# XiandaGuo/OpenStereo

Measured on NVIDIA H100. Metric: stereo_pairs_per_sec_gwcnet_256x512_d192, higher is better.
Workload: dtype f32

## Files before the change

### include/openstereo_b200.h

```cpp
#ifndef OPENSTEREO_B200_H_
#define OPENSTEREO_B200_H_

#include <stddef.h>
#include <stdint.h>

#ifdef __cplusplus
extern "C" {
#endif

#define OSB_OK 0
#define OSB_EINVAL 1
#define OSB_ECUDA 2
#define OSB_EUNSUPPORTED 3

#define OSB_ACT_NONE 0
#define OSB_ACT_RELU 1
#define OSB_ACT_LEAKY 2
#define OSB_ACT_RELU6 3

typedef void* osb_stream_t;

int osb_abi_version(void);
const char* osb_last_error(void);
uint64_t osb_launch_count(void);
// ... 39 lines not shown

int osb_deconv3d_bn_act_fwd(const float* x, const float* w_packed, const float* scale,
                            const float* shift, const float* residual, float* y, int B, int Cin,
                            int Cout, int D, int H, int W, int kernel, int act, osb_stream_t stream);

int osb_conv3d_1x1_bn_act_fwd(const float* x0, const float* x1, int Cin0, const float* w_packed,
                              const float* scale, const float* shift, const float* residual,
                              const float* gate, float* y, int B, int Cin, int Cout, int D, int H,
                              int W, int act, int sigmoid_out, osb_stream_t stream);


int osb_conv3d_tc_supported(int Cin, int Cout, int W, int stride);
#define OSB_TC_MIN_WIDTH 24
int osb_tc_general_width(int W);
int osb_conv3d_tc_kc(int Cin, int Cout, int W, int stride);
int osb_conv3d_k3_tc_fwd(const float* x_ndhwc, const void* w_split, const float* scale, const float* shift,
                         const float* residual, float* y, int B, int Cin, int Cout, int D, int H, int W, int act,
                         int out_ndhwc, int res_ndhwc, osb_stream_t stream);
int osb_conv3d_k3_tc_gate_fwd(const float* x_ndhwc, const void* w_split, const float* scale, const float* shift,
                              const float* residual, const float* gate_nhwc, float* y, int B, int Cin, int Cout, int D, int H, int W,
                              int act, osb_stream_t stream);
int osb_conv3d_k3_tc_ncdhw_fwd(const float* x_ncdhw, const void* w_split, const float* scale, const float* shift,
                               const float* residual, float* y, int B, int Cin, int Cout, int D, int H, int W, int act,
                               int out_ndhwc, int res_ndhwc, osb_stream_t stream);
int osb_conv3d_s2_tc_supported(int Cin, int Cout, int D, int H, int W);
int osb_conv3d_k3_s2_tc_fwd(const float* x_ndhwc, const void* w_split, const float* scale, const float* shift,
                            const float* residual, float* y, int B, int Cin, int Cout, int D, int H, int W, int act,
                            int out_ndhwc, int res_ndhwc, osb_stream_t stream);
int osb_deconv3d_tc_supported(int Cin, int Cout, int W);
int osb_deconv3d_k3_tc_fwd(const float* x_ndhwc, const void* w_split, const float* scale, const float* shift,
                           const float* residual, float* y, int B, int Cin, int Cout, int D, int H, int W, int act,
                           int out_ndhwc, int res_ndhwc, osb_stream_t stream);
int osb_deconv3d_k4_tc_supported(int Cin, int Cout, int W);
int osb_deconv3d_k4_tc_fwd(const float* x_ndhwc, const void* w_split, const float* scale, const float* shift,
                           const float* residual, float* y, int B, int Cin, int Cout, int cout_real, int D, int H, int W, int act,
                           int out_ndhwc, int res_ndhwc, osb_stream_t stream);
int osb_conv3d_k3_tc_cs_fwd(const float* x_ndhwc, const void* w_split, const float* scale, const float* shift, const float* residual,
                            const float* gate_nhwc, float* y, int B, int Cin, int Cout, int D, int H, int W, int act, int ystride,
                            osb_stream_t stream);
int osb_conv3d_k3_s2_tc_cs_fwd(const float* x_ndhwc, const void* w_split, const float* scale, const float* shift, float* y, int B,
                               int Cin, int Cout, int D, int H, int W, int act, int ystride, osb_stream_t stream);
int osb_deconv3d_k4_tc_cs_fwd(const float* x_ndhwc, const void* w_split, const float* scale, const float* shift, float* y, int B,
                              int Cin, int Cout, int D, int H, int W, int act, int ystride, osb_stream_t stream);
int osb_conv1x1_ndhwc_cat_fwd(const float* x0, const float* x1, int C0, int C1, const float* w_packed, const float* scale,
                              const float* shift, float* y, long long voxels, int Cout, int act, osb_stream_t stream);
int osb_conv1x1_ndhwc_fwd(const float* x, const float* w_packed, const float* scale, const float* shift, float* y,
                          long long voxels, int Cin, int Cout, int act, osb_stream_t stream);
int osb_conv3d_k3_c1_ndhwc_fwd(const float* x_ndhwc, const float* w_taps, const float* scale, const float* shift, float* y, int B,
                               int Cin, int D, int H, int W, osb_stream_t stream);
int osb_conv2d_tc_kc(int Cin, int Cout, int W, int dilation);
int osb_conv2d_k3_tc_fwd(const float* x_nhwc, const void* w_split, const float* scale, const float* shift, const float* residual,
                         float* y, int B, int Cin, int Cout, int H, int W, int dilation, int act, int out_nhwc, int res_nhwc,
                         osb_stream_t stream);
int osb_gwc_volume_sum_fwd(const float* ref, const float* tgt, float* out, int B, int C, int H, int W, int D, int G,
                           osb_stream_t stream);
int osb_group_l2_normalize_fwd(const float* x, float* y, int B, int C, int H, int W, int G, float eps, osb_stream_t stream);
int osb_sub_volume_fwd(const float* left, const float* right, float* out, int B, int C, int H, int W, int D, osb_stream_t stream);
int osb_regression_values_fwd(const float* prob, const float* values, float* out, int B, int D, int H, int W, osb_stream_t stream);

int osb_warped_concat_volume_fwd(const float* x, const float* y, const float* disp, float* out, int B, int C, int D, int H, int W,
                                 int mask_left, osb_stream_t stream);
int osb_warped_gwc_concat_volume_fwd(const float* xg, const float* yg, const float* xc, const float* yc, const float* disp,
                                     float* out, int B, int Cg, int G, int Cc, int D, int H, int W, osb_stream_t stream);

int osb_coex_regression_fwd(const float* cost, const float* spx, float* out, int B, int D, int h, int w, int top_k, int spx_is_logits,
                            osb_stream_t stream);
int osb_nearest_resize3d_fwd(const float* x, float* y, int N, int Di, int Hi, int Wi, int Do, int Ho, int Wo, osb_stream_t stream);

int osb_mbv2_block3d_fwd(const float* x, const float* w_exp, const float* scale1, const float* shift1, const float* w_dw,
                         const float* scale2, const float* shift2, const float* w_proj, const float* scale3, const float* shift3,
                         const float* residual, float* y, int B, int Cin, int Chid, int Cout, int D, int H, int W, int stride,
                         int in_layout, int out_layout, osb_stream_t stream);

int osb_gwc_volume_bwd(const float* grad_vol, const float* ref, const float* tgt, float* grad_ref, float* grad_tgt, int B, int C,
                       int H, int W, int D, int G, int reduce_sum, osb_stream_t stream);
int osb_concat_volume_bwd(const float* grad_vol, float* grad_ref, float* grad_tgt, int B, int C, int H, int W, int D, int mask_left,
                          osb_stream_t stream);
int osb_softargmin_bwd(const float* cost, const float* grad_out, float* grad_cost, int B, int D, int H, int W, float alpha,
                       float start, float step, int normalize, osb_stream_t stream);

int osb_dwconv2d_fwd(const float* x, const float* w, const float* scale, const float* shift, const float* residual, float* y, int B,
                     int C, int H, int W, int KH, int KW, int stride, int act, osb_stream_t stream);
int osb_deconv2d_k3s2_fwd(const float* x, const float* w_packed, const float* scale, const float* shift, const float* residual,
                          float* y, int B, int Cin, int Cout, int H, int W, int act, osb_stream_t stream);

int osb_avgpool_pairs_fwd(const float* x, float* y, long long outer, int n, long long inner, osb_stream_t stream);
int osb_geo_lookup_fwd(const float* geo0, const float* geo1, const float* geo2, const float* geo3, const float* corr0,
                       const float* corr1, const float* corr2, const float* corr3, const float* disp, const float* coords,
                       float* out, int B, int C, int D, int H, int W, int W2, int num_levels, int radius, osb_stream_t stream);
int osb_context_upsample_fwd(const float* disp_low, const float* up_weights, float* out, int B, int h, int w, int scale,
                             osb_stream_t stream);
int osb_ncdhw_to_ndhwc(const float* x, float* y, int B, int C, int D, int H, int W, osb_stream_t stream);
int osb_ncdhw_to_ndhwc_pad(const float* x, float* y, int B, int C, int Cpad, int D, int H, int W, osb_stream_t stream);
int osb_feature_att_gate_fwd(const float* feat_nchw, const float* w1_packed, const float* scale1, const float* shift1,
                             const float* w2_packed, const float* scale2, const float* shift2, float* gate_nhwc, int B,
                             int Cf, int Ch, int Cv, int Cpad, int HW, int act1, osb_stream_t stream);

#ifdef __cplusplus
}
#endif
#endif
```

### openstereo_b200/_lib.py

```python
import ctypes
import os

_PKG = os.path.dirname(os.path.abspath(__file__))
LIB_PATH = os.path.join(_PKG, "lib", "libopenstereo_b200.so")

_f32p = ctypes.c_void_p
_i = ctypes.c_int
_f = ctypes.c_float
_s = ctypes.c_void_p

SIGNATURES = {
    "osb_gwc_volume_fwd": [_f32p, _f32p, _f32p, _i, _i, _i, _i, _i, _i, _s],
    "osb_concat_volume_fwd": [_f32p, _f32p, _f32p, _i, _i, _i, _i, _i, _i, _s],
    "osb_gwc_concat_volume_fwd": [_f32p, _f32p, _f32p, _f32p, _f32p, _i, _i, _i, _i, _i, _i, _i, _s],
    "osb_corr_volume_fwd": [_f32p, _f32p, _f32p, _i, _i, _i, _i, _i, _s],
    "osb_softargmin_fwd": [_f32p, _f32p, _i, _i, _i, _i, _f, _f, _f, _i, _s],
    "osb_upsample_softargmin_fwd": [_f32p, _f32p, _i, _i, _i, _i, _i, _i, _i, _i, _s],
    "osb_epe_partial_fwd": [_f32p, _f32p, _f32p, _i, _i, _f, _s],
    "osb_conv3d_k3_bn_act_fwd": [_f32p] * 7 + [_i] * 8 + [_s],
    "osb_deconv3d_bn_act_fwd": [_f32p] * 6 + [_i] * 8 + [_s],
    "osb_conv3d_1x1_bn_act_fwd": [_f32p, _f32p, _i] + [_f32p] * 6 + [_i] * 8 + [_s],
    "osb_conv3d_tc_supported": [_i, _i, _i, _i],
    "osb_conv3d_tc_kc": [_i, _i, _i, _i],
    "osb_tc_general_width": [_i],
    "osb_conv3d_s2_tc_supported": [_i, _i, _i, _i, _i],
    "osb_deconv3d_tc_supported": [_i, _i, _i],
    "osb_deconv3d_k3_tc_fwd": [_f32p] * 6 + [_i] * 9 + [_s],
    "osb_conv3d_k3_s2_tc_fwd": [_f32p] * 6 + [_i] * 9 + [_s],
    "osb_conv3d_k3_tc_fwd": [_f32p] * 6 + [_i] * 9 + [_s],
    "osb_conv3d_k3_tc_ncdhw_fwd": [_f32p] * 6 + [_i] * 9 + [_s],
    "osb_conv3d_k3_tc_gate_fwd": [_f32p] * 7 + [_i] * 7 + [_s],
    "osb_deconv3d_k4_tc_supported": [_i, _i, _i],
    "osb_conv3d_k3_tc_cs_fwd": [_f32p] * 7 + [_i] * 8 + [_s],
    "osb_conv3d_k3_s2_tc_cs_fwd": [_f32p] * 5 + [_i] * 8 + [_s],
    "osb_deconv3d_k4_tc_cs_fwd": [_f32p] * 5 + [_i] * 8 + [_s],
    "osb_deconv3d_k4_tc_fwd": [_f32p] * 6 + [_i] * 10 + [_s],
    "osb_conv1x1_ndhwc_cat_fwd": [_f32p, _f32p, _i, _i, _f32p, _f32p, _f32p, _f32p, ctypes.c_longlong, _i, _i, _s],
    "osb_feature_att_gate_fwd": [_f32p] * 8 + [_i] * 7 + [_s],
    "osb_ncdhw_to_ndhwc_pad": [_f32p, _f32p, _i, _i, _i, _i, _i, _i, _s],
    "osb_conv1x1_ndhwc_fwd": [_f32p] * 5 + [ctypes.c_longlong, _i, _i, _i, _s],
    "osb_conv3d_k3_c1_ndhwc_fwd": [_f32p] * 5 + [_i] * 5 + [_s],
    "osb_avgpool_pairs_fwd": [_f32p, _f32p, ctypes.c_longlong, _i, ctypes.c_longlong, _s],
    "osb_geo_lookup_fwd": [_f32p] * 11 + [_i] * 8 + [_s],
    "osb_context_upsample_fwd": [_f32p] * 3 + [_i] * 4 + [_s],
    "osb_conv2d_tc_kc": [_i] * 4,
    "osb_conv2d_k3_tc_fwd": [_f32p] * 6 + [_i] * 9 + [_s],
    "osb_ncdhw_to_ndhwc": [_f32p, _f32p, _i, _i, _i, _i, _i, _s],
    "osb_gwc_volume_sum_fwd": [_f32p, _f32p, _f32p, _i, _i, _i, _i, _i, _i, _s],
    "osb_group_l2_normalize_fwd": [_f32p, _f32p, _i, _i, _i, _i, _i, _f, _s],
    "osb_sub_volume_fwd": [_f32p, _f32p, _f32p, _i, _i, _i, _i, _i, _s],
    "osb_regression_values_fwd": [_f32p, _f32p, _f32p, _i, _i, _i, _i, _s],
    "osb_gwc_volume_bwd": [_f32p] * 5 + [_i] * 7 + [_s],
    "osb_concat_volume_bwd": [_f32p] * 3 + [_i] * 6 + [_s],
    "osb_softargmin_bwd": [_f32p] * 3 + [_i] * 4 + [_f, _f, _f, _i, _s],
    "osb_dwconv2d_fwd": [_f32p] * 6 + [_i] * 8 + [_s],
    "osb_deconv2d_k3s2_fwd": [_f32p] * 6 + [_i] * 6 + [_s],
    "osb_upsample_softargmin_values_fwd": [_f32p] * 3 + [_i] * 8 + [_s],
    "osb_warped_concat_volume_fwd": [_f32p] * 4 + [_i] * 6 + [_s],
    "osb_warped_gwc_concat_volume_fwd": [_f32p] * 6 + [_i] * 7 + [_s],
    "osb_coex_regression_fwd": [_f32p] * 3 + [_i] * 6 + [_s],
    "osb_nearest_resize3d_fwd": [_f32p] * 2 + [_i] * 7 + [_s],
    "osb_mbv2_block3d_fwd": [_f32p] * 12 + [_i] * 10 + [_s],
}


class NativeLibraryError(RuntimeError):
    pass


def _load():
    if not os.path.exists(LIB_PATH):
        raise NativeLibraryError(
            "%s not found: build it with `python -m openstereo_b200.build` (there is no CPU/PyTorch fallback)"
            % LIB_PATH)
    lib = ctypes.CDLL(LIB_PATH)
    lib.osb_abi_version.restype = ctypes.c_int
    lib.osb_last_error.restype = ctypes.c_char_p
    lib.osb_launch_count.restype = ctypes.c_uint64
    lib.osb_tc_overflow_count.argtypes = [ctypes.c_void_p, ctypes.c_int, ctypes.POINTER(ctypes.c_uint)]
    lib.osb_tc_overflow_count.restype = ctypes.c_int
    lib.osb_tc_overflow_poll.argtypes = [ctypes.c_void_p, ctypes.c_void_p]
    lib.osb_tc_overflow_poll.restype = ctypes.c_int
    lib.osb_tc_overflow_flag.argtypes = []
    lib.osb_tc_overflow_flag.restype = ctypes.c_void_p
    lib.osb_set_rz_kappa.argtypes = [ctypes.c_float]
    lib.osb_set_rz_kappa.restype = ctypes.c_float
    lib.osb_set_persistent_grid_cap.argtypes = [ctypes.c_int]
    lib.osb_set_persistent_grid_cap.restype = ctypes.c_int
    lib.osb_tc_last_variant.argtypes = []
    lib.osb_tc_last_variant.restype = ctypes.c_char_p
    for name, argtypes in SIGNATURES.items():
        try:
            fn = getattr(lib, name)
        except AttributeError as exc:
            raise NativeLibraryError("%s does not export %s" % (LIB_PATH, name)) from exc
        fn.argtypes = argtypes
        fn.restype = ctypes.c_int
    return lib

# ... 18 lines not shown
```

### openstereo_b200/csrc/conv3d_tcs2.cu

```cuda
#include "tc_common.cuh"

namespace osb {

struct Tcs2Params {
  const float* x;
  const void* w;
  const float* scale;
  const float* shift;
  const float* residual;
  float* y;
  int B, D, H, Cin;
  int act;
  float kappa;
  unsigned int* overflow;
  int out_ndhwc, res_ndhwc;
  int items, hblocks;
  int Wr, ctiles;
  int ystride;
};

template <int COUT, int KC, int W, int TILES, bool GW = false>
struct Tcs2Cfg {
  static_assert(!GW || W == 128, "general-width tiles are 128-column segments of one output row");
  static constexpr int HALO = GW ? 1 : 0;
  static constexpr int CSTEP = 128 - HALO;
  static constexpr int R = 128 / W;
  static constexpr int ROWB = KC * 4;
  static constexpr int UNIT_BYTES = 128 * ROWB;
  static constexpr int N3 = 3 * COUT;
  static constexpr int G = 32;
  static constexpr int NG = COUT / G;
  static constexpr int NP = (NG + TC_WGS - 1) / TC_WGS;
  static constexpr int B_SLICE = N3 * ROWB;
  static constexpr int B_SUB = 3 * G * ROWB;
  static constexpr int B_SLOT = TC_WGS * B_SUB;
  static constexpr int PC = 16;
  static constexpr int NPASS = G / PC;
  static constexpr int LD = 3 * PC + 4;
  static constexpr int XCHG_FLOATS = 2 * 4 * PC;
  static constexpr int NLW = 4;
  static constexpr int FIXED_SMEM = 1024 + TC_BSLOTS * 3 * B_SLOT + TC_WGS * 128 * LD * 4 + 1024 + TC_WGS * XCHG_FLOATS * 4 + 3 * COUT * 4;
  static constexpr int STAGES = (232448 - FIXED_SMEM) / UNIT_BYTES < 10 ? (232448 - FIXED_SMEM) / UNIT_BYTES : 10;
  static_assert(STAGES >= NLW, "the ring must hold at least one unit per loader warp");
  static constexpr int NU = TILES * 3 * 2;
  static constexpr int HBLK = TILES * R;
  static constexpr int KSTEPS = KC / 16;
  static constexpr int LO = KC / 8;
  static constexpr int A_OFF = 0;
  static constexpr int B_OFF = A_OFF + STAGES * UNIT_BYTES;
  static constexpr int STAGE_OFF = B_OFF + TC_BSLOTS * 3 * B_SLOT;
  static constexpr int BAR_OFF = STAGE_OFF + TC_WGS * 128 * LD * 4;
  static constexpr int THREADS = TC_WG_THREADS;
  static constexpr size_t SMEM = 1024 + (size_t)BAR_OFF + 1024 + TC_WGS * XCHG_FLOATS * 4 + 3 * COUT * 4;
  static_assert(SMEM <= 232448, "shared memory budget of one CTA exceeded");
  static_assert(TILES == 1, "a consumer warpgroup holds one accumulator tile");
  static_assert(COUT % G == 0, "output channels come in groups of 32");
  static_assert(32 * LD >= TP_WARP_FLOATS, "store_ndhwc_chunk32 transposes through the warp's own rows of the staging tile");
  static_assert(B_SUB % 1024 == 0 && UNIT_BYTES % 1024 == 0, "operand tiles must stay 1024-byte aligned");
};

template <int N>
__device__ __forceinline__ void s2_stage16(float* stage, int ld, const float (&acc)[2][N / 2], int c0, int dst, int wq, int lane) {
#pragma unroll
  for (int h = 0; h < 2; ++h) {
// ... 8 lines not shown
}

template <int COUT, int KC, int W, int TILES, bool GW = false>
__global__ void __launch_bounds__(Tcs2Cfg<COUT, KC, W, TILES, GW>::THREADS, 1) conv3d_tcs2_kernel(const Tcs2Params p) {
  using C = Tcs2Cfg<COUT, KC, W, TILES, GW>;
  extern __shared__ __align__(1024) uint8_t smem_raw[];
  uint8_t* smem = smem_raw + ((1024u - (smem_u32(smem_raw) & 1023u)) & 1023u);
  uint8_t* a_buf = smem + C::A_OFF;
  uint8_t* b_buf = smem + C::B_OFF;
  float* stage = reinterpret_cast<float*>(smem + C::STAGE_OFF);
  uint64_t* bars = reinterpret_cast<uint64_t*>(smem + C::BAR_OFF);
  uint64_t* a_ready = bars;
  uint64_t* a_empty = a_ready + C::STAGES;
  uint64_t* b_full = a_empty + C::STAGES;
  uint64_t* b_empty = b_full + TC_BSLOTS * 3;
  float* xchg = reinterpret_cast<float*>(smem + C::BAR_OFF + 1024);
  float* s_scale = xchg + TC_WGS * C::XCHG_FLOATS;
  float* s_shift = s_scale + COUT;
  float* zeros = s_shift + COUT;

  const int warp = threadIdx.x >> 5, lane = threadIdx.x & 31;
  const int nchunk = p.Cin / KC;
  const int Wp = GW ? p.Wr : W;
  const int YS = (W < 32 && p.ystride) ? p.ystride : COUT;
  const int ctiles = GW ? p.ctiles : 1;

  if (threadIdx.x == 0) {
    for (int s = 0; s < C::STAGES; ++s) {
      mbar_init(&a_ready[s], 32);
      mbar_init(&a_empty[s], 4 * TC_WGS);
    }
    for (int k = 0; k < TC_BSLOTS * 3; ++k) {
      mbar_init(&b_full[k], 1);
      mbar_init(&b_empty[k], 4 * TC_WGS);
    }
    fence_mbar_init();
  }
  for (int c = threadIdx.x; c < COUT; c += blockDim.x) {
    s_scale[c] = p.scale ? p.scale[c] : 1.f;
    s_shift[c] = p.shift ? p.shift[c] : 0.f;
    zeros[c] = 0.f;
  }
  __syncthreads();

  if (warp < 4 * TC_WGS) {
    setmaxnreg_inc<TC_CONSUMER_REGS>();
    const int wg = warp >> 2;
    stage += wg * 128 * C::LD;
    xchg += wg * C::XCHG_FLOATS;
    const int bar_stage = 1 + 2 * wg, bar_xchg = 2 + 2 * wg;
    const uint64_t dbase = (KC == 32) ? desc_sw128_base() : desc_sw64_base();
    constexpr uint32_t A_HALF = 64 * C::ROWB / 16;
    const uint32_t b16 = (smem_u32(b_buf) & 0x3FFFF) >> 4;
    const int Do = p.D / 2, Ho = p.H / 2;
    const int q = warp & 3;
    const int m = q * 32 + lane;
    const int rr = m / W, wcol = m % W;
    const bool has_left_q = ((q * 32) % W) != 0;
    uint32_t unitc = 0, phc = 0, exc = 0;
    for (int it = blockIdx.x; it < p.items; it += gridDim.x) {
      const int g = (it % C::NP) * TC_WGS + wg;
      const bool has_group = g < C::NG;
      const int cg = g * C::G;
      const int it0 = it / C::NP;
      const int ct = it0 % ctiles;
      const int hb = (it0 / ctiles) % p.hblocks;
      const int d = (it0 / (ctiles * p.hblocks)) % Do;
      const int b = it0 / (ctiles * p.hblocks * Do);
      float acc_e[2][C::G / 2], acc_o[2][C::G];
      uint32_t accum_e = 0, accum_o = 0;
      for (int kd = 0; kd < 3; ++kd) {
        const int din = 2 * d + kd - 1;
        if (din < 0 || din >= p.D) continue;
        for (int ch = 0; ch < nchunk; ++ch, ++phc) {
#pragma unroll
          for (int kh = 0; kh < 3; ++kh) {
            const uint32_t bslot = (phc & 1) * 3 + kh;
#pragma unroll
            for (int par = 0; par < 2; ++par) {
              const uint32_t slot = unitc % C::STAGES, ph = (unitc / C::STAGES) & 1;
              mbar_wait(&a_ready[slot], ph);
              if (par == 0) mbar_wait(&b_full[bslot], (phc >> 1) & 1);
              if (has_group) {
                const uint64_t da0 = dbase | (uint64_t)((smem_u32(a_buf + slot * C::UNIT_BYTES) & 0x3FFFF) >> 4);
                const uint64_t db0 = dbase | (uint64_t)(b16 + (bslot * C::B_SLOT + wg * C::B_SUB + (par ? C::G * C::ROWB : 0)) / 16);
                wg_fence();
#pragma unroll
                for (int ks = 0; ks < C::KSTEPS; ++ks) {
                  if (par == 0) wg_mma_split<C::G>(acc_e, da0 + 2 * ks, A_HALF, db0 + 2 * ks, C::LO, ks > 0 ? 1u : accum_e);
                  else wg_mma_split<2 * C::G>(acc_o, da0 + 2 * ks, A_HALF, db0 + 2 * ks, C::LO, ks > 0 ? 1u : accum_o);
                }
                wg_commit();
                wg_wait_all();
                if (par == 0) accum_e = 1;
                else accum_o = 1;
              }
              wg_release(&a_empty[slot], lane);
              if (par == 1) wg_release(&b_empty[bslot], lane);
              ++unitc;
            }
          }
        }
      }
      if (!has_group) continue;
      const int h = hb * C::HBLK + rr;
      const bool live = h < Ho;
      const int col = GW ? ct * C::CSTEP - C::HALO + m : wcol;
// ... 37 lines not shown
            out[pass * C::PC + i0 + k] = ((left + p1[k]) + p2[k]) * corr;
          }
        }
      }
      const uint32_t vm = (W < 32) ? __ballot_sync(0xffffffffu, live) : (live ? vmask : 0u);
      if (vm && p.out_ndhwc && (!p.residual || p.res_ndhwc)) {
        store_ndhwc_chunk32(stage + q * 32 * C::LD, lane, out, p.y + (vox - lane) * YS + cg,
                            p.residual ? p.residual + (vox - lane) * YS + cg : nullptr, YS, s_scale + cg, s_shift + cg, p.act, vm);
      } else if (live && cvalid) {
#pragma unroll
        for (int i = 0; i < 32; ++i) out[i] = fmaf(out[i], s_scale[cg + i], s_shift[cg + i]);
        if (p.residual) {
          if (p.res_ndhwc) {
            const float4* rp = reinterpret_cast<const float4*>(p.residual + vox * YS + cg);
#pragma unroll
            for (int i = 0; i < 8; ++i) {
              const float4 rv = __ldg(rp + i);
              out[4 * i] += rv.x, out[4 * i + 1] += rv.y, out[4 * i + 2] += rv.z, out[4 * i + 3] += rv.w;
            }
          } else {
#pragma unroll
            for (int i = 0; i < 32; ++i) out[i] += __ldg(p.residual + ncdhw0 + (size_t)(cg + i) * plane);
          }
        }
        if (p.act == OSB_ACT_RELU) {
#pragma unroll
          for (int i = 0; i < 32; ++i) out[i] = fmaxf(out[i], 0.f);
        } else if (p.act == OSB_ACT_LEAKY) {
#pragma unroll
          for (int i = 0; i < 32; ++i) out[i] = out[i] > 0.f ? out[i] : 0.01f * out[i];
        }
        if (p.out_ndhwc) {
          float4* yp = reinterpret_cast<float4*>(p.y + vox * YS + cg);
#pragma unroll
          for (int i = 0; i < 8; ++i) yp[i] = make_float4(out[4 * i], out[4 * i + 1], out[4 * i + 2], out[4 * i + 3]);
        } else {
#pragma unroll
          for (int i = 0; i < 32; ++i) p.y[ncdhw0 + (size_t)(cg + i) * plane] = out[i];
        }
      }
    }
  }
  else if (warp < 4 * TC_WGS + C::NLW) {
    setmaxnreg_dec<TC_LOADER_REGS>();
    const int lw = warp - 4 * TC_WGS;
    static_assert(KC == 16, "lane_voxel / unit-row mapping below is written for 64-byte operand rows");
    constexpr int CPR = KC / 4;
    constexpr int VPL = 32 / CPR;
    constexpr int NLD = 128 / VPL;
    static_assert(W % VPL == 0, "a load instruction must not straddle image rows");
    const int v0 = lane_voxel<KC>(lane), c = lane % CPR;
    float amax = 0.f;
    const int WI = 2 * Wp;
    const int Do = p.D / 2;
    uint32_t ubase = 0;
    int first = lw;
    auto fill = [&](const float* base, size_t rstride, size_t cstride, int h_first, int h_step, uint32_t u, int col0) {
      float4 v[NLD];
#pragma unroll
      for (int j = 0; j < NLD; ++j) {
        const int hin = h_first + h_step * ((VPL * j) / W);
        const size_t off = (size_t)((VPL * j) / W) * rstride + (size_t)((VPL * j) % W) * cstride;
        bool ok = hin >= 0 && hin < p.H;
        if (GW) ok = ok && (unsigned)(col0 + VPL * j) < (unsigned)Wp;
        v[j] = ok ? __ldg(reinterpret_cast<const float4*>(base + (ptrdiff_t)off)) : make_float4(0.f, 0.f, 0.f, 0.f);
      }
      const uint32_t slot = u % C::STAGES, ph = (u / C::STAGES) & 1;
      mbar_wait_relaxed(&a_empty[slot], ph ^ 1);
      uint8_t* tile = a_buf + slot * C::UNIT_BYTES;
#pragma unroll
      for (int j = 0; j < NLD; ++j) stage_f16_split<KC>(tile, v0 + VPL * j, c, v[j], amax);
      fence_proxy_async();
      mbar_arrive(&a_ready[slot]);
    };
    for (int it = blockIdx.x; it < p.items; it += gridDim.x) {
      const int it0 = it / C::NP;
      const int ct = it0 % ctiles;
      const int hb = (it0 / ctiles) % p.hblocks;
      const int od = (it0 / (ctiles * p.hblocks)) % Do;
      const int b = it0 / (ctiles * p.hblocks * Do);
      const int h0 = hb * C::HBLK;
      const int col0 = ct * C::CSTEP - C::HALO + v0;
      for (int kd = 0; kd < 3; ++kd) {
        const int din = 2 * od + kd - 1;
        if (din < 0 || din >= p.D) continue;
        const float* plane = p.x + ((size_t)b * p.D + din) * p.H * (size_t)WI * p.Cin;
        for (int ch = 0; ch < nchunk; ++ch) {
#pragma unroll 1
          for (int j = first; j < C::NU; j += C::NLW) {
            const int t = j / 6, kh = (j >> 1) % 3, par = j & 1;
            const int h_first = 2 * (h0 + t * C::R) + kh - 1;
            const float* base = plane + ((ptrdiff_t)h_first * WI + 2 * col0 + par) * p.Cin + ch * KC + c * 4;
            fill(base, (size_t)2 * WI * p.Cin, (size_t)2 * p.Cin, h_first, 2, ubase + j, col0);
          }
          ubase += C::NU;
          first = (first + C::NLW - C::NU % C::NLW) % C::NLW;
        }
      }
    }
    tc_report_overflow(p.overflow, amax);
  }
  else {
    setmaxnreg_dec<TC_PRODUCER_REGS>();
    if (warp == 4 * TC_WGS + C::NLW && elect_one()) {
      const uint8_t* wsrc = reinterpret_cast<const uint8_t*>(p.w);
      uint32_t phc = 0;
      for (int it = blockIdx.x; it < p.items; it += gridDim.x) {
        const int g0 = (it % C::NP) * TC_WGS;
        const int ngr = min(TC_WGS, C::NG - g0);
        const int od = (it / C::NP / (ctiles * p.hblocks)) % (p.D / 2);
        for (int kd = 0; kd < 3; ++kd) {
          const int din = 2 * od + kd - 1;
          if (din < 0 || din >= p.D) continue;
          for (int ch = 0; ch < nchunk; ++ch, ++phc) {
            for (int kh = 0; kh < 3; ++kh) {
              const uint32_t slot = (phc & 1) * 3 + kh;
              const size_t slice = ((size_t)kd * nchunk + ch) * 3 + kh;
              mbar_wait_relaxed(&b_empty[slot], ((phc >> 1) & 1) ^ 1);
              mbar_arrive_expect_tx(&b_full[slot], ngr * C::B_SUB);
              for (int t = 0; t < ngr; ++t)
#pragma unroll
                for (int kw = 0; kw < 3; ++kw)
                  bulk_g2s(b_buf + slot * C::B_SLOT + t * C::B_SUB + kw * C::G * C::ROWB,
                           wsrc + slice * C::B_SLICE + (size_t)(kw * COUT + (g0 + t) * C::G) * C::ROWB, C::G * C::ROWB, &b_full[slot]);
            }
          }
        }
      }
    }
    __syncwarp();
  }
}

template <int COUT, int KC, int W, int TILES, bool GW = false>
static int launch_tcs2(const TcArgs& a, cudaStream_t stream) {
  using C = Tcs2Cfg<COUT, KC, W, TILES, GW>;
  Tcs2Params p{};
  p.ystride = a.ystride;
  p.hblocks = (a.H / 2 + C::HBLK - 1) / C::HBLK;
  p.Wr = GW ? a.W / 2 : W;
  p.ctiles = GW ? (p.Wr + C::CSTEP - 1) / C::CSTEP : 1;
  static const std::string variant = tc_variant_name("tcs2<%d,%d,%d,%d,%d>", COUT, KC, W, TILES, (int)GW);
  return launch_persistent<conv3d_tcs2_kernel<COUT, KC, W, TILES, GW>>(
      a, p, (long long)a.B * (a.D / 2) * p.hblocks * p.ctiles * C::NP, C::SMEM, variant.c_str(), stream);
}

static TcLaunch select_conv3d_s2_tc(int Cin, int Cout, int D, int H, int W, bool slice) {
  if (Cin % 16 != 0 || Cin < 16 || D % 2 || H % 2 || W % 2) return nullptr;
  if (W == 32 && Cout == 96) return launch_tcs2<96, 16, 16, 1>;
  if (W == 32 && Cout == 64) return launch_tcs2<64, 16, 16, 1>;
  if (slice) return nullptr;
  if (W == 128 && Cout == 64) return launch_tcs2<64, 16, 64, 1>;
  if (W == 64 && Cout == 64) return launch_tcs2<64, 16, 32, 1>;
  if (W == 64 && Cout == 128) return launch_tcs2<128, 16, 32, 1>;
  if (W == 64 && Cout == 96) return launch_tcs2<96, 16, 32, 1>;
  if (!osb_tc_general_width(W / 2)) return nullptr;
  if (Cout == 64) return launch_tcs2<64, 16, 128, 1, true>;
  if (Cout == 128) return launch_tcs2<128, 16, 128, 1, true>;
  return nullptr;
}

static int conv3d_k3_s2_tc_impl(TcArgs a, cudaStream_t stream) {
  OSB_REQUIRE(select_conv3d_s2_tc(a.Cin, a.Cout, a.D, a.H, a.W, false), "conv3d_k3_s2_tc: unsupported shape Cin=%d Cout=%d D=%d H=%d W=%d",
              a.Cin, a.Cout, a.D, a.H, a.W);
  const TcLaunch launch = select_conv3d_s2_tc(a.Cin, a.Cout, a.D, a.H, a.W, a.slice());
  const int rc = check_tc_args("conv3d_k3_s2_tc", a, launch);
  return rc != OSB_OK ? rc : launch(a, stream);
}

}

extern "C" {

int osb_conv3d_s2_tc_supported(int Cin, int Cout, int D, int H, int W) {
  return osb::select_conv3d_s2_tc(Cin, Cout, D, H, W, false) ? 1 : 0;
}

int osb_conv3d_k3_s2_tc_fwd(const float* x_ndhwc, const void* w_split, const float* scale, const float* shift,
                            const float* residual, float* y, int B, int Cin, int Cout, int D, int H, int W, int act,
                            int out_ndhwc, int res_ndhwc, osb_stream_t stream) {
  return osb::conv3d_k3_s2_tc_impl({x_ndhwc, w_split, scale, shift, residual, nullptr, y, B, Cin, Cout, D, H, W, act, out_ndhwc, res_ndhwc,
                                    0, 0, Cout}, (cudaStream_t)stream);
}

int osb_conv3d_k3_s2_tc_cs_fwd(const float* x_ndhwc, const void* w_split, const float* scale, const float* shift, float* y, int B,
                               int Cin, int Cout, int D, int H, int W, int act, int ystride, osb_stream_t stream) {
  return osb::conv3d_k3_s2_tc_impl({x_ndhwc, w_split, scale, shift, nullptr, nullptr, y, B, Cin, Cout, D, H, W, act, 1, 1, 0, ystride,
                                    Cout}, (cudaStream_t)stream);
}
}
```

### openstereo_b200/host_models.py

```python
import torch
import torch.nn as nn
import torch.nn.functional as F

from . import aggregation as _agg
from . import ops
from .aggregation import GwcAggregation, PSMAggregation


USE_TC_BACKBONE = True


def _cfg_get(cfgs, key, default=None):
    if isinstance(cfgs, dict):
        return cfgs.get(key, default)
    return getattr(cfgs, key, default)


def _cb(cin, cout, k, stride, pad, dilation, bias=False):
    return nn.Sequential(nn.Conv2d(cin, cout, kernel_size=k, stride=stride, padding=dilation if dilation > 1 else pad,
                                   dilation=dilation, bias=bias), nn.BatchNorm2d(cout))


def _front_tc_ok(net, x):
    return (getattr(net, "_osb_folded", False) and x.is_cuda and x.dim() == 4 and x.shape[2] == 2 * ops.TC_WIDTH and x.shape[3] % 2 == 0
            and _agg.USE_TENSOR_CORES and USE_TC_BACKBONE and x.dtype == torch.float32 and ops.conv3d_tc_kc(32, 32, ops.TC_WIDTH) == 32)


def _front_tc(net, x):
    convs = [m for m in net.firstconv.modules() if isinstance(m, nn.Conv2d)]
    blocks = list(net.layer1.children())
    y = F.relu(convs[0](x))
    t = y.permute(0, 3, 2, 1).contiguous()
    t = _tc2d(net, convs[2], _tc2d(net, convs[1], t, ops.ACT_RELU, transpose=True), ops.ACT_RELU, transpose=True)
    for i, blk in enumerate(blocks):
        c1, c2 = _block_convs(blk)
        assert blk.downsample is None
        t = _tc2d(net, c2, _tc2d(net, c1, t, ops.ACT_RELU, transpose=True), ops.ACT_NONE, residual=t, last=(i == len(blocks) - 1),
                  transpose=True)
    return t.transpose(2, 3).contiguous()


def _tc2d(net, conv, t, act, residual=None, last=False, transpose=False):
    cache = net.__dict__.setdefault("_osb_tc2d", {})
    dil = conv.dilation[0]
    if id(conv) not in cache:
        assert conv.kernel_size == (3, 3) and conv.stride == (1, 1) and conv.padding == (dil, dil) and conv.dilation == (dil, dil)
        w5 = torch.zeros(conv.out_channels, conv.in_channels, 3, 3, 3, dtype=torch.float32, device=conv.weight.device)
        w2 = conv.weight.detach().float()
        w5[:, :, 1] = w2.transpose(2, 3) if transpose else w2
        kc = ops.conv2d_tc_kc(conv.in_channels, conv.out_channels, ops.TC_WIDTH, dil)
        cache[id(conv)] = (ops.pack_tc_weight(w5, kc), None if conv.bias is None else conv.bias.detach().float().contiguous())
    wp, bias = cache[id(conv)]
    return ops.conv2d_k3_tc(t, wp, None, bias, residual, act, dil, out_nhwc=not last, res_nhwc=True)


def _block_convs(blk):
    c1 = [m for m in blk.conv1.modules() if isinstance(m, nn.Conv2d)][0]
    c2 = [m for m in blk.conv2.modules() if isinstance(m, nn.Conv2d)][0]
    return c1, c2


def _block_tc_ok(blk, c):
    if blk.downsample is not None:
        return False
    c1, c2 = _block_convs(blk)
    dil = c1.dilation[0]
    return all(cv.kernel_size == (3, 3) and cv.stride == (1, 1) and cv.dilation == (dil, dil) and cv.padding == (dil, dil)
               and cv.in_channels == c and cv.out_channels == c for cv in (c1, c2)) and ops.conv2d_tc_kc(c, c, ops.TC_WIDTH, dil) != 0


def _stage_tc(net, stage, x):
    blocks = list(stage.children())
    usable = getattr(net, "_osb_folded", False) and x.is_cuda and x.dtype == torch.float32 and _agg.USE_TENSOR_CORES and USE_TC_BACKBONE
    y, rest = x, blocks
    if not (usable and x.shape[3] == ops.TC_WIDTH and _block_tc_ok(blocks[0], x.shape[1])):
        y, rest = blocks[0](x), blocks[1:]
    c = y.shape[1]
    if not (usable and rest and y.shape[3] == ops.TC_WIDTH and all(_block_tc_ok(b, c) for b in rest)):
        for b in rest:
            y = b(y)
        return y
    t = ops.to_ndhwc(y.unsqueeze(2).contiguous()).squeeze(1)
    for i, b in enumerate(rest):
        c1, c2 = _block_convs(b)
        t = _tc2d(net, c2, _tc2d(net, c1, t, ops.ACT_RELU), ops.ACT_NONE, residual=t, last=(i == len(rest) - 1))
    return t


def _lastconv_tc_ok(net, x):
    convs = [m for m in net.lastconv.modules() if isinstance(m, nn.Conv2d)]
    return (getattr(net, "_osb_folded", False) and x.is_cuda and x.dtype == torch.float32 and _agg.USE_TENSOR_CORES and USE_TC_BACKBONE
            and x.shape[3] == ops.TC_WIDTH and len(convs) == 2 and convs[0].kernel_size == (3, 3) and convs[0].stride == (1, 1)
            and convs[0].dilation == (1, 1) and convs[0].padding == (1, 1) and convs[1].kernel_size == (1, 1)
            and ops.conv2d_tc_kc(convs[0].in_channels, convs[0].out_channels, ops.TC_WIDTH, 1) != 0)


def _lastconv_tc(net, x):
    convs = [m for m in net.lastconv.modules() if isinstance(m, nn.Conv2d)]
    t = ops.to_ndhwc(x.unsqueeze(2).contiguous()).squeeze(1)
    return convs[1](_tc2d(net, convs[0], t, ops.ACT_RELU, last=True))


def gwc_extract(net, x):
    x = _front_tc(net, x) if _front_tc_ok(net, x) else net.layer1(net.firstconv(x))
    l2 = _stage_tc(net, net.layer2, x)
    l3 = _stage_tc(net, net.layer3, l2)
    l4 = _stage_tc(net, net.layer4, l3)
    gwc = torch.cat((l2, l3, l4), dim=1)
    out = {"gwc_feature": gwc}
    if net.concat_feature:
        out["concat_feature"] = _lastconv_tc(net, gwc) if _lastconv_tc_ok(net, gwc) else net.lastconv(gwc)
    return out


def psm_extract(net, x):
    o2 = _front_tc(net, x) if _front_tc_ok(net, x) else net.layer1(net.firstconv(x))
    o4_0 = _stage_tc(net, net.layer2, o2)
    o8 = _stage_tc(net, net.layer4, _stage_tc(net, net.layer3, o4_0))
    size = (o8.size()[2], o8.size()[3])
    up = [F.interpolate(getattr(net, "branch%d" % i)(o8), size, mode="bilinear", align_corners=True) for i in (1, 2, 3, 4)]
    cat = torch.cat((o4_0, o8, up[3], up[2], up[1], up[0]), 1)
    return _lastconv_tc(net, cat) if _lastconv_tc_ok(net, cat) else net.lastconv(cat)


class _ResBlock(nn.Module):

    def __init__(self, conv1, conv2, downsample):
        super().__init__()
        self.conv1, self.conv2, self.downsample = conv1, conv2, downsample

    def forward(self, x):
        out = self.conv2(self.conv1(x))
        if self.downsample is not None:
            x = self.downsample(x)
        out += x
        return out


def _stage(make_block, make_down, inplanes, planes, blocks, stride):
    down = make_down(inplanes, planes, stride) if (stride != 1 or inplanes != planes) else None
    layers = [make_block(inplanes, planes, stride, down)]
    layers += [make_block(planes, planes, 1, None) for _ in range(1, blocks)]
    return nn.Sequential(*layers)


class _GwcFeatureExtraction(nn.Module):
    def __init__(self, concat_feature, concat_channels):
        super().__init__()
        self.concat_feature = concat_feature
        r = lambda: nn.ReLU(inplace=True)
        self.firstconv = nn.Sequential(_cb(3, 32, 3, 2, 1, 1), r(), _cb(32, 32, 3, 1, 1, 1), r(), _cb(32, 32, 3, 1, 1, 1), r())

        def block(dil):
            return lambda i, o, s, d: _ResBlock(nn.Sequential(_cb(i, o, 3, s, 1, dil), r()), _cb(o, o, 3, 1, 1, dil), d)

        down = lambda i, o, s: nn.Sequential(nn.Conv2d(i, o, kernel_size=1, stride=s, bias=False), nn.BatchNorm2d(o))
        self.layer1 = _stage(block(1), down, 32, 32, 3, 1)
        self.layer2 = _stage(block(1), down, 32, 64, 16, 2)
        self.layer3 = _stage(block(1), down, 64, 128, 3, 1)
        self.layer4 = _stage(block(2), down, 128, 128, 3, 1)
        if concat_feature:
            self.lastconv = nn.Sequential(_cb(320, 128, 3, 1, 1, 1), r(),
                                          nn.Conv2d(128, concat_channels, kernel_size=1, padding=0, stride=1, bias=False))

    def forward(self, x):
        return gwc_extract(self, x)


def _fold_conv_bn(module):
    import copy
    from torch.nn.utils.fusion import fuse_conv_bn_eval
    inst_fwd = module.__dict__.pop("forward", None)
    try:
        fused = copy.deepcopy(module).eval()
    finally:
# ... 238 lines not shown
```

### openstereo_b200/ops.py

```python
import math

import torch

from . import _lib

ACT_NONE, ACT_RELU, ACT_LEAKY, ACT_RELU6 = 0, 1, 2, 3
TC_WIDTH = 128
TC_KC = 32


_LAUNCH_DEVICE = [None]


def _stream(t):
    _LAUNCH_DEVICE[0] = t.device.index
    return torch.cuda.current_stream(t.device).cuda_stream


def _same_device(*tensors):
    devs = {t.device for t in tensors if t is not None}
    if len(devs) > 1:
        raise RuntimeError("openstereo_b200: operands live on different devices: %s" % sorted(str(d) for d in devs))


# ... 812 lines not shown
    outer, inner = math.prod(x.shape[:axis]), math.prod(x.shape[axis + 1:])
    y = torch.empty(x.shape[:axis] + (n // 2,) + x.shape[axis + 1:], dtype=torch.float32, device=x.device)
    _call("osb_avgpool_pairs_fwd", x.data_ptr(), y.data_ptr(), outer, n, inner, _stream(y))
    return y


def geo_lookup(geo_levels, corr_levels, disp, coords, radius):
    levels = len(geo_levels)
    assert levels == len(corr_levels) and 1 <= levels <= 4
    b, c, d, h, w = geo_levels[0].shape
    w2 = corr_levels[0].shape[-1]
    for i in range(levels):
        g, cr = geo_levels[i], corr_levels[i]
        assert g.is_cuda and g.dtype == torch.float32 and g.is_contiguous() and tuple(g.shape) == (b, c, d >> i, h, w)
        assert cr.is_cuda and cr.dtype == torch.float32 and cr.is_contiguous() and tuple(cr.shape) == (b, h, w, w2 >> i)
    disp = disp.contiguous().float()
    coords = coords.reshape(b, h, w).contiguous().float()
    assert tuple(disp.shape) == (b, 1, h, w)
    out = torch.empty((b, levels * (c + 1) * (2 * radius + 1), h, w), dtype=torch.float32, device=disp.device)
    gp = [geo_levels[i].data_ptr() if i < levels else None for i in range(4)]
    cp = [corr_levels[i].data_ptr() if i < levels else None for i in range(4)]
    _call("osb_geo_lookup_fwd", *gp, *cp, disp.data_ptr(), coords.data_ptr(), out.data_ptr(), b, c, d, h, w, w2, levels, radius,
          _stream(out))
    return out


def context_upsample(disp_low, up_weights, scale_factor=4):
    assert disp_low.is_cuda and disp_low.dim() == 4 and disp_low.shape[1] == 1
    b, _, h, w = disp_low.shape
    assert tuple(up_weights.shape) == (b, 9, h * scale_factor, w * scale_factor)
    disp_low, up_weights = disp_low.contiguous().float(), up_weights.contiguous().float()
    out = torch.empty((b, h * scale_factor, w * scale_factor), dtype=torch.float32, device=disp_low.device)
    _call("osb_context_upsample_fwd", disp_low.data_ptr(), up_weights.data_ptr(), out.data_ptr(), b, h, w, scale_factor, _stream(out))
    return out


def conv2d_tc_kc(cin, cout, w, dilation=1):
    return int(_lib.lib.osb_conv2d_tc_kc(int(cin), int(cout), int(w), int(dilation)))


def conv2d_k3_tc(x_nhwc, w_split, scale=None, shift=None, residual=None, act=ACT_NONE, dilation=1, out_nhwc=True, res_nhwc=True):
    assert x_nhwc.is_cuda and x_nhwc.dtype == torch.float32 and x_nhwc.is_contiguous() and x_nhwc.dim() == 4
    b, h, w, cin = x_nhwc.shape
    cout = w_split.cout
    kc = conv2d_tc_kc(cin, cout, w, dilation)
    assert kc
    wptr, scale = _tc_args(w_split, cin, kc, scale)
    y = torch.empty((b, h, w, cout) if out_nhwc else (b, cout, h, w), dtype=torch.float32, device=x_nhwc.device)
    if residual is not None:
        assert residual.is_contiguous() and residual.numel() == y.numel()
    _call("osb_conv2d_k3_tc_fwd", x_nhwc.data_ptr(), wptr, _ptr(scale), _ptr(shift), _ptr(residual), y.data_ptr(), b, cin,
          cout, h, w, dilation, act, int(out_nhwc), int(res_nhwc), _stream(y))
    return y
```

Measured before the change: 282.8.

## Run GwcNet feature extractor channels-last end to end with stride-2 TC conv

Adds a 2D stride-2 tensor-core conv entry point that reuses the 3D stride-2 kernel with D=1. It also adds a channels-last path through the GwcNet backbone: the front stage stays NHWC, entry blocks use the new s2 conv, and the downsample is computed as a linear on the strided view. The path concatenates features in NHWC and only permutes once for the gwc output. This removes repeated NCHW/NHWC transposes and the fallback PyTorch convs in the layer2/layer3 entry blocks. The cost is extra dispatch logic and a new D=1 case in the s2 kernel.

```diff
diff --git a/include/openstereo_b200.h b/include/openstereo_b200.h
--- a/include/openstereo_b200.h
+++ b/include/openstereo_b200.h
@@ -115,6 +115,8 @@
 int osb_conv2d_k3_tc_fwd(const float* x_nhwc, const void* w_split, const float* scale, const float* shift, const float* residual,
                          float* y, int B, int Cin, int Cout, int H, int W, int dilation, int act, int out_nhwc, int res_nhwc,
                          osb_stream_t stream);
+int osb_conv2d_k3_s2_tc_fwd(const float* x_nhwc, const void* w_split, const float* scale, const float* shift, const float* residual,
+                            float* y, int B, int Cin, int Cout, int H, int W, int act, int out_nhwc, int res_nhwc, osb_stream_t stream);
 int osb_gwc_volume_sum_fwd(const float* ref, const float* tgt, float* out, int B, int C, int H, int W, int D, int G,
                            osb_stream_t stream);
 int osb_group_l2_normalize_fwd(const float* x, float* y, int B, int C, int H, int W, int G, float eps, osb_stream_t stream);
diff --git a/openstereo_b200/_lib.py b/openstereo_b200/_lib.py
--- a/openstereo_b200/_lib.py
+++ b/openstereo_b200/_lib.py
@@ -45,6 +45,7 @@
     "osb_context_upsample_fwd": [_f32p] * 3 + [_i] * 4 + [_s],
     "osb_conv2d_tc_kc": [_i] * 4,
     "osb_conv2d_k3_tc_fwd": [_f32p] * 6 + [_i] * 9 + [_s],
+    "osb_conv2d_k3_s2_tc_fwd": [_f32p] * 6 + [_i] * 8 + [_s],
     "osb_ncdhw_to_ndhwc": [_f32p, _f32p, _i, _i, _i, _i, _i, _s],
     "osb_gwc_volume_sum_fwd": [_f32p, _f32p, _f32p, _i, _i, _i, _i, _i, _i, _s],
     "osb_group_l2_normalize_fwd": [_f32p, _f32p, _i, _i, _i, _i, _i, _f, _s],
diff --git a/openstereo_b200/csrc/conv3d_tcs2.cu b/openstereo_b200/csrc/conv3d_tcs2.cu
--- a/openstereo_b200/csrc/conv3d_tcs2.cu
+++ b/openstereo_b200/csrc/conv3d_tcs2.cu
@@ -10,6 +10,7 @@
   const float* residual;
   float* y;
   int B, D, H, Cin;
+  int Do;
   int act;
   float kappa;
   unsigned int* overflow;
@@ -124,7 +125,7 @@
     const uint64_t dbase = (KC == 32) ? desc_sw128_base() : desc_sw64_base();
     constexpr uint32_t A_HALF = 64 * C::ROWB / 16;
     const uint32_t b16 = (smem_u32(b_buf) & 0x3FFFF) >> 4;
-    const int Do = p.D / 2, Ho = p.H / 2;
+    const int Do = p.Do, Ho = p.H / 2;
     const int q = warp & 3;
     const int m = q * 32 + lane;
     const int rr = m / W, wcol = m % W;
@@ -268,7 +269,7 @@
     const int v0 = lane_voxel<KC>(lane), c = lane % CPR;
     float amax = 0.f;
     const int WI = 2 * Wp;
-    const int Do = p.D / 2;
+    const int Do = p.Do;
     uint32_t ubase = 0;
     int first = lw;
     auto fill = [&](const float* base, size_t rstride, size_t cstride, int h_first, int h_step, uint32_t u, int col0) {
@@ -324,7 +325,7 @@
       for (int it = blockIdx.x; it < p.items; it += gridDim.x) {
         const int g0 = (it % C::NP) * TC_WGS;
         const int ngr = min(TC_WGS, C::NG - g0);
-        const int od = (it / C::NP / (ctiles * p.hblocks)) % (p.D / 2);
+        const int od = (it / C::NP / (ctiles * p.hblocks)) % p.Do;
         for (int kd = 0; kd < 3; ++kd) {
           const int din = 2 * od + kd - 1;
           if (din < 0 || din >= p.D) continue;
@@ -353,16 +354,17 @@
   using C = Tcs2Cfg<COUT, KC, W, TILES, GW>;
   Tcs2Params p{};
   p.ystride = a.ystride;
+  p.Do = a.D == 1 ? 1 : a.D / 2;
   p.hblocks = (a.H / 2 + C::HBLK - 1) / C::HBLK;
   p.Wr = GW ? a.W / 2 : W;
   p.ctiles = GW ? (p.Wr + C::CSTEP - 1) / C::CSTEP : 1;
   static const std::string variant = tc_variant_name("tcs2<%d,%d,%d,%d,%d>", COUT, KC, W, TILES, (int)GW);
   return launch_persistent<conv3d_tcs2_kernel<COUT, KC, W, TILES, GW>>(
-      a, p, (long long)a.B * (a.D / 2) * p.hblocks * p.ctiles * C::NP, C::SMEM, variant.c_str(), stream);
+      a, p, (long long)a.B * p.Do * p.hblocks * p.ctiles * C::NP, C::SMEM, variant.c_str(), stream);
 }
 
 static TcLaunch select_conv3d_s2_tc(int Cin, int Cout, int D, int H, int W, bool slice) {
-  if (Cin % 16 != 0 || Cin < 16 || D % 2 || H % 2 || W % 2) return nullptr;
+  if (Cin % 16 != 0 || Cin < 16 || (D % 2 && D != 1) || H % 2 || W % 2) return nullptr;
   if (W == 32 && Cout == 96) return launch_tcs2<96, 16, 16, 1>;
   if (W == 32 && Cout == 64) return launch_tcs2<64, 16, 16, 1>;
   if (slice) return nullptr;
@@ -399,6 +401,12 @@
                                     0, 0, Cout}, (cudaStream_t)stream);
 }
 
+int osb_conv2d_k3_s2_tc_fwd(const float* x_nhwc, const void* w_split, const float* scale, const float* shift, const float* residual,
+                            float* y, int B, int Cin, int Cout, int H, int W, int act, int out_nhwc, int res_nhwc, osb_stream_t stream) {
+  return osb::conv3d_k3_s2_tc_impl({x_nhwc, w_split, scale, shift, residual, nullptr, y, B, Cin, Cout, 1, H, W, act, out_nhwc, res_nhwc,
+                                    0, 0, Cout}, (cudaStream_t)stream);
+}
+
 int osb_conv3d_k3_s2_tc_cs_fwd(const float* x_ndhwc, const void* w_split, const float* scale, const float* shift, float* y, int B,
                                int Cin, int Cout, int D, int H, int W, int act, int ystride, osb_stream_t stream) {
   return osb::conv3d_k3_s2_tc_impl({x_ndhwc, w_split, scale, shift, nullptr, nullptr, y, B, Cin, Cout, D, H, W, act, 1, 1, 0, ystride,
diff --git a/openstereo_b200/host_models.py b/openstereo_b200/host_models.py
--- a/openstereo_b200/host_models.py
+++ b/openstereo_b200/host_models.py
@@ -26,7 +26,7 @@
             and _agg.USE_TENSOR_CORES and USE_TC_BACKBONE and x.dtype == torch.float32 and ops.conv3d_tc_kc(32, 32, ops.TC_WIDTH) == 32)
 
 
-def _front_tc(net, x):
+def _front_tc(net, x, nhwc=False):
     convs = [m for m in net.firstconv.modules() if isinstance(m, nn.Conv2d)]
     blocks = list(net.layer1.children())
     y = F.relu(convs[0](x))
@@ -35,22 +35,27 @@
     for i, blk in enumerate(blocks):
         c1, c2 = _block_convs(blk)
         assert blk.downsample is None
-        t = _tc2d(net, c2, _tc2d(net, c1, t, ops.ACT_RELU, transpose=True), ops.ACT_NONE, residual=t, last=(i == len(blocks) - 1),
-                  transpose=True)
-    return t.transpose(2, 3).contiguous()
+        t = _tc2d(net, c2, _tc2d(net, c1, t, ops.ACT_RELU, transpose=True), ops.ACT_NONE, residual=t,
+                  last=(i == len(blocks) - 1 and not nhwc), transpose=True)
+    return t if nhwc else t.transpose(2, 3).contiguous()
 
 
 def _tc2d(net, conv, t, act, residual=None, last=False, transpose=False):
     cache = net.__dict__.setdefault("_osb_tc2d", {})
-    dil = conv.dilation[0]
-    if id(conv) not in cache:
-        assert conv.kernel_size == (3, 3) and conv.stride == (1, 1) and conv.padding == (dil, dil) and conv.dilation == (dil, dil)
+    dil, s = conv.dilation[0], conv.stride[0]
+    key = (id(conv), s)
+    if key not in cache:
+        assert conv.kernel_size == (3, 3) and conv.stride == (s, s) and conv.padding == (dil, dil) and conv.dilation == (dil, dil)
+        assert s == 1 or (s == 2 and dil == 1)
         w5 = torch.zeros(conv.out_channels, conv.in_channels, 3, 3, 3, dtype=torch.float32, device=conv.weight.device)
         w2 = conv.weight.detach().float()
         w5[:, :, 1] = w2.transpose(2, 3) if transpose else w2
-        kc = ops.conv2d_tc_kc(conv.in_channels, conv.out_channels, ops.TC_WIDTH, dil)
-        cache[id(conv)] = (ops.pack_tc_weight(w5, kc), None if conv.bias is None else conv.bias.detach().float().contiguous())
-    wp, bias = cache[id(conv)]
+        wp = (ops.pack_tc_weight(w5, 16, kw_order=(1, 0, 2)) if s == 2 else
+              ops.pack_tc_weight(w5, ops.conv2d_tc_kc(conv.in_channels, conv.out_channels, ops.TC_WIDTH, dil)))
+        cache[key] = (wp, None if conv.bias is None else conv.bias.detach().float().contiguous())
+    wp, bias = cache[key]
+    if s == 2:
+        return ops.conv2d_k3_s2_tc(t, wp, None, bias, residual, act, out_nhwc=not last, res_nhwc=True)
     return ops.conv2d_k3_tc(t, wp, None, bias, residual, act, dil, out_nhwc=not last, res_nhwc=True)
 
 
@@ -80,11 +85,60 @@
         for b in rest:
             y = b(y)
         return y
-    t = ops.to_ndhwc(y.unsqueeze(2).contiguous()).squeeze(1)
-    for i, b in enumerate(rest):
+    return _blocks_tc(net, rest, _nhwc(y), last=True)
+
+
+def _nhwc(x):
+    return ops.to_ndhwc(x.unsqueeze(2).contiguous()).squeeze(1)
+
+
+def _blocks_tc(net, blocks, t, last=False):
+    for i, b in enumerate(blocks):
         c1, c2 = _block_convs(b)
-        t = _tc2d(net, c2, _tc2d(net, c1, t, ops.ACT_RELU), ops.ACT_NONE, residual=t, last=(i == len(rest) - 1))
+        t = _tc2d(net, c2, _tc2d(net, c1, t, ops.ACT_RELU), ops.ACT_NONE, residual=t, last=last and i == len(blocks) - 1)
     return t
+
+
+def _entry_block_ok(blk, cin, cout, stride):
+    down = list(blk.downsample.children()) if blk.downsample is not None else []
+    if not (len(down) == 1 and isinstance(down[0], nn.Conv2d) and down[0].kernel_size == (1, 1) and down[0].padding == (0, 0)
+            and down[0].stride == (stride, stride) and down[0].in_channels == cin and down[0].out_channels == cout):
+        return False
+    c1, c2 = _block_convs(blk)
+    return all(cv.kernel_size == (3, 3) and cv.stride == (s, s) and cv.dilation == (1, 1) and cv.padding == (1, 1)
+               and (cv.in_channels, cv.out_channels) == io for cv, s, io in ((c1, stride, (cin, cout)), (c2, 1, (cout, cout))))
+
+
+def _entry_tc(net, blk, t, transpose=False):
+    c1, c2 = _block_convs(blk)
+    down = list(blk.downsample.children())[0]
+    s = down.stride[0]
+    r = F.linear(t[:, ::s, ::s] if s > 1 else t, down.weight.view(down.out_channels, down.in_channels), down.bias)
+    return _tc2d(net, c2, _tc2d(net, c1, t, ops.ACT_RELU, transpose=transpose), ops.ACT_NONE, residual=r, transpose=transpose)
+
+
+def _entry_tc_ok(net, x):
+    if not (_front_tc_ok(net, x) and x.shape[3] == 4 * ops.TC_WIDTH):
+        return False
+    l2, l3, l4 = (list(s.children()) for s in (net.layer2, net.layer3, net.layer4))
+    return (_entry_block_ok(l2[0], 32, 64, 2) and _entry_block_ok(l3[0], 64, 128, 1)
+            and ops.conv3d_s2_tc_supported(32, 64, 1, x.shape[3] // 2, ops.TC_WIDTH) and ops.conv2d_tc_kc(64, 64, ops.TC_WIDTH // 2) == 16
+            and ops.conv2d_tc_kc(64, 128, ops.TC_WIDTH) == 16
+            and all(_block_tc_ok(b, 64) for b in l2[1:]) and all(_block_tc_ok(b, 128) for b in l3[1:] + l4))
+
+
+def _gwc_extract_cl(net, x):
+    l2b, l3b = list(net.layer2.children()), list(net.layer3.children())
+    t = _entry_tc(net, l2b[0], _front_tc(net, x, nhwc=True), transpose=True)
+    l2 = _blocks_tc(net, l2b[1:], t.transpose(1, 2).contiguous())
+    l3 = _blocks_tc(net, l3b[1:], _entry_tc(net, l3b[0], l2))
+    l4 = _blocks_tc(net, list(net.layer4.children()), l3)
+    gwc_cl = torch.cat((l2, l3, l4), dim=3)
+    gwc = gwc_cl.permute(0, 3, 1, 2).contiguous()
+    out = {"gwc_feature": gwc}
+    if net.concat_feature:
+        out["concat_feature"] = _lastconv_tc(net, gwc_cl) if _lastconv_tc_ok(net, gwc) else net.lastconv(gwc)
+    return out
 
 
 def _lastconv_tc_ok(net, x):
@@ -95,13 +149,14 @@
             and ops.conv2d_tc_kc(convs[0].in_channels, convs[0].out_channels, ops.TC_WIDTH, 1) != 0)
 
 
-def _lastconv_tc(net, x):
+def _lastconv_tc(net, t):
     convs = [m for m in net.lastconv.modules() if isinstance(m, nn.Conv2d)]
-    t = ops.to_ndhwc(x.unsqueeze(2).contiguous()).squeeze(1)
     return convs[1](_tc2d(net, convs[0], t, ops.ACT_RELU, last=True))
 
 
 def gwc_extract(net, x):
+    if _entry_tc_ok(net, x):
+        return _gwc_extract_cl(net, x)
     x = _front_tc(net, x) if _front_tc_ok(net, x) else net.layer1(net.firstconv(x))
     l2 = _stage_tc(net, net.layer2, x)
     l3 = _stage_tc(net, net.layer3, l2)
@@ -109,7 +164,7 @@
     gwc = torch.cat((l2, l3, l4), dim=1)
     out = {"gwc_feature": gwc}
     if net.concat_feature:
-        out["concat_feature"] = _lastconv_tc(net, gwc) if _lastconv_tc_ok(net, gwc) else net.lastconv(gwc)
+        out["concat_feature"] = _lastconv_tc(net, _nhwc(gwc)) if _lastconv_tc_ok(net, gwc) else net.lastconv(gwc)
     return out
 
 
@@ -120,7 +175,7 @@
     size = (o8.size()[2], o8.size()[3])
     up = [F.interpolate(getattr(net, "branch%d" % i)(o8), size, mode="bilinear", align_corners=True) for i in (1, 2, 3, 4)]
     cat = torch.cat((o4_0, o8, up[3], up[2], up[1], up[0]), 1)
-    return _lastconv_tc(net, cat) if _lastconv_tc_ok(net, cat) else net.lastconv(cat)
+    return _lastconv_tc(net, _nhwc(cat)) if _lastconv_tc_ok(net, cat) else net.lastconv(cat)
 
 
 class _ResBlock(nn.Module):
diff --git a/openstereo_b200/ops.py b/openstereo_b200/ops.py
--- a/openstereo_b200/ops.py
+++ b/openstereo_b200/ops.py
@@ -888,3 +888,17 @@
     _call("osb_conv2d_k3_tc_fwd", x_nhwc.data_ptr(), wptr, _ptr(scale), _ptr(shift), _ptr(residual), y.data_ptr(), b, cin,
           cout, h, w, dilation, act, int(out_nhwc), int(res_nhwc), _stream(y))
     return y
+
+
+def conv2d_k3_s2_tc(x_nhwc, w_split, scale=None, shift=None, residual=None, act=ACT_NONE, out_nhwc=True, res_nhwc=True):
+    assert x_nhwc.is_cuda and x_nhwc.dtype == torch.float32 and x_nhwc.is_contiguous() and x_nhwc.dim() == 4
+    b, h, w, cin = x_nhwc.shape
+    cout = w_split.cout
+    wptr, scale = _tc_args(w_split, cin, 16, scale)
+    ho, wo = h // 2, w // 2
+    y = torch.empty((b, ho, wo, cout) if out_nhwc else (b, cout, ho, wo), dtype=torch.float32, device=x_nhwc.device)
+    if residual is not None:
+        assert tuple(residual.shape) == ((b, ho, wo, cout) if res_nhwc else (b, cout, ho, wo)) and residual.is_contiguous()
+    _call("osb_conv2d_k3_s2_tc_fwd", x_nhwc.data_ptr(), wptr, _ptr(scale), _ptr(shift), _ptr(residual), y.data_ptr(), b, cin,
+          cout, h, w, act, int(out_nhwc), int(res_nhwc), _stream(y))
+    return y
```

After: 300.5 (median of 6 runs). +6.3%, better.
